# GlassyWing/yolo_deepsort

Measured on AMD Instinct MI355X. Metric: end-to-end frames/sec (detect+ReID+assoc), 608x608, higher is better.
Workload: dtype f16x3

## Files before the change

yolo_deepsort_amd/csrc/conv_bench.cpp:

```cpp
#include "conv_common.h"
#include "conv_weights.h"
#include "h16.h"

#include <algorithm>
#include <math.h>
#include <stdlib.h>
#include <string.h>

namespace yds {
namespace {

uint16_t f16_bits_saturating(float x) {
    const float xs = x * H16_A_SCALE;
    _Float16 h = (_Float16)xs;
    if (isfinite(xs) && !isfinite((float)h)) h = (_Float16)(xs > 0.f ? 65504.f : -65504.f);
    uint16_t b;
    memcpy(&b, &h, 2);
    return b;
}

struct CaseViews {
    int x_ld, x_off, y_ld, y_off, r_ld, r_off, n_split, y2_ld, y2_off;
};

struct ConvCase {
    ConvArgs a;
    ConvWeights cw;
    DevBuf<float> x, y, y2, res, raw[4];
    View y_whole, y2_whole;

    static void put(View &v, const float *host, DevBuf<float> &raw, DevBuf<float> &packed) {
        if (v.fmt == FMT_F16) {
            const size_t count = v.pixels() * v.c;
            std::vector<uint16_t> h(count);
            for (size_t i = 0; i < count; ++i) h[i] = f16_bits_saturating(host[i]);
            v.ld = fmt_slots(FMT_F16, v.c);
            packed.upload(reinterpret_cast<const float *>(h.data()), count / 2);
            YDS_HIP(hipDeviceSynchronize());
            v.p = packed.p;
            return;
        }
        raw.upload(host, v.pixels() * v.c);
        v.p = raw.p;
        if (v.fmt != FMT_H16) return;
        packed.alloc(raw.n);
        v.p = packed.p;
        launch_pack_h16(raw.p, v, nullptr);
    }
    static View slice(const View &whole, int off, int c) {
        View v = whole;
        v.p = whole.p + fmt_slots(whole.fmt, off);
        v.c = c;
        return v;
    }
    static bool h16_ok(int c, int ld, int off) { return c % 32 == 0 && ld % 32 == 0 && off % 32 == 0; }
    ConvCase(int n, int h, int w, int cin, int cout, int ksize, int stride, int act, const float *x_nhwc, const float *w_okkc, const float *bias,
             const float *res_nhwc, int res_mode, const CaseViews *vw = nullptr, float sentinel = 0.f, int fmt_x = 0, int fmt_y = 0) {
        const int pad = (ksize - 1) / 2, ho = (h + 2 * pad - ksize) / stride + 1, wo = (w + 2 * pad - ksize) / stride + 1;
        const CaseViews d = vw ? *vw : CaseViews{cin, 0, (cout + 3) / 4 * 4, 0, cout, 0, 0, 0, 0};
        const bool f16 = conv_math() == MATH_F16X3;
        const int c1 = d.n_split > 0 ? d.n_split : cout, c2 = cout - c1;
        cw.shape(cout, cin, cin, ksize, stride, pad);
        cw.upload_korder(w_okkc, bias, nullptr);
        cw.fill(a);
        a.act = act;
        View x_whole{nullptr, n, h, w, d.x_ld, d.x_ld, fmt_x == FMT_F16 ? FMT_F16 : (f16 && h16_ok(cin, d.x_ld, d.x_off)) ? FMT_H16 : FMT_F32};
        const int yfmt = fmt_y == FMT_F16 ? FMT_F16 : (f16 && h16_ok(c1, d.y_ld, d.y_off) && h16_ok(c2, d.y2_ld, d.y2_off)) ? FMT_H16 : FMT_F32;
        y_whole = View{nullptr, n, ho, wo, d.y_ld, d.y_ld, yfmt};
        if (x_nhwc) put(x_whole, x_nhwc, raw[0], x);
        else x_whole.ld = fmt_slots(x_whole.fmt, d.x_ld);
        a.x = slice(x_whole, d.x_off, cin);
        if (vw) {
            const std::vector<float> fill(y_whole.pixels() * (size_t)std::max(d.y_ld, d.y2_ld), sentinel);
            put(y_whole, fill.data(), raw[2], y);
            if (c2 > 0) {
                y2_whole = View{nullptr, n, ho, wo, d.y2_ld, d.y2_ld, yfmt};
                put(y2_whole, fill.data(), raw[3], y2);
                a.y2 = slice(y2_whole, d.y2_off, c2);
                a.n_split = c1;
            }
        } else {
            y_whole.ld = fmt_slots(yfmt, d.y_ld);
            y.alloc(y_whole.pixels() * y_whole.ld);
            y_whole.p = y.p;
        }
        a.y = slice(y_whole, d.y_off, cout);
        if (res_mode) {
            View r_whole{nullptr, n, ho, wo, d.r_ld, d.r_ld, yfmt};
            put(r_whole, res_nhwc, raw[1], res);
            a.res = slice(r_whole, d.r_off, cout);
            a.res_mode = res_mode;
        }
        YDS_HIP(hipDeviceSynchronize());
    }
};

}
}

extern "C" {

int yds_conv_bench(int n, int h, int w, int cin, int cout, int ksize, int stride, int act, int with_residual, int iters, double *avg_us,
                   int *variant) {
    YDS_API_BEGIN
    using namespace yds;
    std::vector<float> hx((size_t)n * h * w * cin), hw((size_t)cout * ksize * ksize * cin), hb(cout);
    unsigned s = 12345u;
    auto rnd = [&]() { s = s * 1664525u + 1013904223u; return ((s >> 8) & 0xffff) / 32768.f - 1.f; };
    const char *dk = getenv("YDS_BENCH_DATA");
    const int data_kind = !dk ? 0 : (!strcmp(dk, "zero") ? 1 : (!strcmp(dk, "const") ? 2 : 0));
    for (auto &v : hx) v = data_kind == 1 ? 0.f : data_kind == 2 ? 0.5f : rnd();
    for (auto &v : hw) v = data_kind == 1 ? 0.f : data_kind == 2 ? 0.03125f : rnd() * 0.05f;
    for (auto &v : hb) v = rnd();
    const int pad = (ksize - 1) / 2;
    const std::vector<float> hr(with_residual ? (size_t)n * ((h + 2 * pad - ksize) / stride + 1) * ((w + 2 * pad - ksize) / stride + 1) * cout : 0, 0.f);
    ConvCase c(n, h, w, cin, cout, ksize, stride, act, hx.data(), hw.data(), hb.data(), hr.data(), with_residual ? RES_AFTER_ACT : RES_NONE);
    if (const char *t = getenv("YDS_BENCH_TERMS")) c.a.terms = atoi(t) == 1 ? 1 : 3;
    hipStream_t st;
    YDS_HIP(hipStreamCreate(&st));
    hipEvent_t e0, e1;
    YDS_HIP(hipEventCreate(&e0)); YDS_HIP(hipEventCreate(&e1));
    int tuned = conv_autotune(c.a, st, nullptr);
    for (int i = 0; i < 3; ++i) *variant = launch_conv(c.a, st, tuned);
    YDS_HIP(hipEventRecord(e0, st));
    for (int i = 0; i < iters; ++i) launch_conv(c.a, st, tuned);
    YDS_HIP(hipEventRecord(e1, st));
    YDS_HIP(hipEventSynchronize(e1));
    float ms = 0;
    YDS_HIP(hipEventElapsedTime(&ms, e0, e1));
    *avg_us = ms * 1e3 / iters;
    (void)hipEventDestroy(e0); (void)hipEventDestroy(e1); (void)hipStreamDestroy(st);
    YDS_API_END
}

int yds_conv_run(int variant, int n, int h, int w, int cin, int cout, int ksize, int stride, int act, int res_mode, const float *x_nhwc,
                 const float *w_okkc, const float *bias, const float *res_nhwc, float *y_nchw) {
    YDS_API_BEGIN
    using namespace yds;
    if (cin % 4) fail("conv_run: input channels must be a multiple of 4");
    if (res_mode && !res_nhwc) fail("conv_run: residual mode %d without a residual tensor", res_mode);
    ConvCase c(n, h, w, cin, cout, ksize, stride, act, x_nhwc, w_okkc, bias, res_nhwc, res_mode);
    launch_conv(c.a, nullptr, variant);
    nhwc_to_host(c.a.y, y_nchw, nullptr);
    YDS_API_END
}

int yds_conv_run_view(int variant, int n, int h, int w, int cin, int cout, int ksize, int stride, int act, int res_mode, const int *view,
                      const float *x_nhwc, const float *w_okkc, const float *bias, const float *res_nhwc, float sentinel, float *y_nchw,
                      float *y2_nchw) {
    YDS_API_BEGIN
    using namespace yds;
    const CaseViews v{view[0], view[1], view[2], view[3], view[4], view[5], view[6], view[7], view[8]};
    const bool merged = v.n_split > 0;
    const int c1 = merged ? v.n_split : cout;
    if (n < 1 || h < 1 || w < 1 || cin < 4 || cout < 1 || cin % 4) fail("conv_run_view: bad shape (input channels must be a multiple of 4)");
    if (res_mode && !res_nhwc) fail("conv_run_view: residual mode %d without a residual tensor", res_mode);
    if (merged && (v.n_split >= cout || res_mode || !y2_nchw)) fail("conv_run_view: a merged launch needs 0 < n_split < cout, a second output and no residual");
    auto inside = [](int off, int c, int ld) { return off >= 0 && c > 0 && off % 4 == 0 && ld % 4 == 0 && off + c <= ld; };
    if (!inside(v.x_off, cin, v.x_ld)) fail("conv_run_view: input slice [%d, %d) does not fit %d channels (multiples of 4)", v.x_off, v.x_off + cin, v.x_ld);
    if (!inside(v.y_off, c1, v.y_ld)) fail("conv_run_view: output slice [%d, %d) does not fit %d channels (multiples of 4)", v.y_off, v.y_off + c1, v.y_ld);
    if (merged && !inside(v.y2_off, cout - c1, v.y2_ld)) fail("conv_run_view: second output slice [%d, %d) does not fit %d channels (multiples of 4)", v.y2_off, v.y2_off + cout - c1, v.y2_ld);
    if (res_mode && !inside(v.r_off, cout, v.r_ld)) fail("conv_run_view: residual slice [%d, %d) does not fit %d channels (multiples of 4)", v.r_off, v.r_off + cout, v.r_ld);
    ConvCase c(n, h, w, cin, cout, ksize, stride, act, x_nhwc, w_okkc, bias, res_nhwc, res_mode, &v, sentinel);
    const int id = variant & kVariantMask;
    if (variant < 0 || id >= kConvVariants) fail("conv_run_view: no such variant %d", variant);
    const std::vector<int> cand = conv_candidates(c.a);
    bool planned = std::find(cand.begin(), cand.end(), id) != cand.end();
    if (id == VAR_SPLITK_64x128 && conv_math() == MATH_F16X3 && !merged && conv_presplit_input(c.a)) {
        const ConvKernelArgs k = make_conv_args(c.a);
        planned = conv_splitk_applicable(k, 0) && conv_splitk_preferred(k);
    }
// ... 88 lines not shown
```

yolo_deepsort_amd/csrc/conv_common.h:

```cpp
#pragma once
#include "common.h"
#include "h16.h"

#include <algorithm>
#include <stdlib.h>
#include <type_traits>

namespace yds {

typedef float f32x16 __attribute__((ext_vector_type(16)));
typedef float f32x4 __attribute__((ext_vector_type(4)));

typedef _Float16 h8 __attribute__((ext_vector_type(8)));
typedef _Float16 h4 __attribute__((ext_vector_type(4)));
constexpr float A_SCALE = 1.f / 256.f, LO_SCALE = 2048.f;
typedef __attribute__((address_space(3))) void lds_void_t;
typedef __attribute__((address_space(1))) const void glb_void_t;
template <int N> __device__ __forceinline__ void wait_vmcnt() { asm volatile("s_waitcnt vmcnt(%0)" ::"n"(N) : "memory"); }

struct ConvKernelArgs {
    const float *x, *w, *bias, *res;
    float *y;
    int H, W, Cin, ldx;
    int Ho, Wo, Cout, ldy, ldr;
    int ksize, stride, pad;
    int K, Kpad, M;
    int act, res_mode;
    int fmt_x, fmt_y, fmt_r;
    int terms;
    int ksplit = 1;
    float *y2 = nullptr;
    int ldy2 = 0, n_split = 0;
    int tiles_m, tiles_n, xm, rm, rn;
    int gn = 1;
    int gn_req = 0;
};

constexpr int KALIGN = 32;
constexpr int STAGGER = 24;

template <int ACT> __device__ __forceinline__ float apply_act(float v) {
    if (ACT == ACT_LEAKY) return v > 0.f ? v : v * 0.1f;
    if (ACT == ACT_RELU) return v > 0.f ? v : 0.f;
    if (ACT == ACT_MISH) {
        const float e = __builtin_amdgcn_exp2f(fminf(v, 20.f) * 1.44269504088896341f);
        const float n = e * (e + 2.f);
        const float m = v * (n * __builtin_amdgcn_rcpf(n + 2.f));
        return v > 20.f ? v : m;
    }
    return v;
}

__device__ __forceinline__ bool tile_of_block(const ConvKernelArgs &p, int &tm, int &tn) {
    const int b = blockIdx.x, xcd = b & 7, idx = b >> 3;
    int lm, ln;
    if (p.gn <= 1) {
        lm = idx % p.rm;
        ln = idx / p.rm;
    } else {
        const int per = p.rm * p.gn, grp = idx / per, w = idx - grp * per;
        const int g = min(p.gn, p.rn - grp * p.gn);
        lm = w / g;
        ln = grp * p.gn + (w - lm * g);
    }
    tm = (xcd % p.xm) * p.rm + lm;
    tn = (xcd / p.xm) * p.rn + ln;
    return tm < p.tiles_m && tn < p.tiles_n;
}

inline int plan_tile_map(ConvKernelArgs &k, int BM, int BN) {
    k.tiles_m = (k.M + BM - 1) / BM;
    k.tiles_n = (k.Cout + BN - 1) / BN;
    long best = -1;
    for (int xm = 1; xm <= 8; xm *= 2) {
        int xn = 8 / xm;
        int rm = (k.tiles_m + xm - 1) / xm, rn = (k.tiles_n + xn - 1) / xn;
        long waste = (long)rm * rn * 8 - (long)k.tiles_m * k.tiles_n;
        long cost = ((long)rm * BM + (long)rn * BN) * 64 + waste * (BM + BN);
        if (best < 0 || cost < best) { best = cost; k.xm = xm; k.rm = rm; k.rn = rn; }
    }
    k.gn = std::max(1, std::min(k.gn_req, k.rn));
    return 8 * k.rm * k.rn;
}

struct FlatRows {
    int m0;
    __device__ __forceinline__ int operator()(int row) const { return m0 + row; }
};
template <int BM, int BN, int WM, int WN, int ACT, int RES, int NT, class RowMap, bool ONE_PASS, class Store>
__device__ __forceinline__ void conv_epilogue_core(const ConvKernelArgs &p, Store store, float *stage, RowMap rows, int n0, int tid) {
    constexpr int ROWS = BM / WM, LD = BN + 4, C4 = BN / 4;
    constexpr int RSTEP = NT / C4;
    static_assert(NT % C4 == 0 && C4 % 2 == 0 && ROWS % RSTEP == 0, "tile width must divide the workgroup; lane pairs share a row");
    const int wave = tid >> 6, wm = wave / WN;
    const int c4 = tid % C4, rr = tid / C4;
    const int n = n0 + c4 * 4;
    const bool n_vec = n + 3 < p.Cout;
    const bool second = p.n_split > 0 && n >= p.n_split;
    float *const y_base = second ? p.y2 : p.y;
    const int y_ld = second ? p.ldy2 : p.ldy, ny = second ? n - p.n_split : n;
    float4 bias4 = make_float4(0.f, 0.f, 0.f, 0.f);
    if (n_vec) bias4 = *reinterpret_cast<const float4 *>(p.bias + n);
    else {
        if (n < p.Cout) bias4.x = p.bias[n];
        if (n + 1 < p.Cout) bias4.y = p.bias[n + 1];
        if (n + 2 < p.Cout) bias4.z = p.bias[n + 2];
    }
    constexpr int PER_PASS = ROWS / RSTEP, NRES = RES != RES_NONE ? WM * PER_PASS : 1;
    auto sweep = [&](auto yf_c, auto rf_c) {
        constexpr int YF = decltype(yf_c)::value, RF = decltype(rf_c)::value;
        constexpr bool YH = YF == FMT_H16, RH = RF == FMT_H16, YS = YF == FMT_F16, RS = RF == FMT_F16;
        float4 rraw[NRES];
        if (RES != RES_NONE) {
#pragma unroll
            for (int q = 0; q < NRES; ++q) {
                const int m = rows((q / PER_PASS) * ROWS + rr + (q % PER_PASS) * RSTEP);
                rraw[q] = make_float4(0.f, 0.f, 0.f, 0.f);
                if (m >= 0 && m < p.M && n < p.Cout) {
                    const float *rp = p.res + (size_t)m * p.ldr;
                    if (RH) {
                        const char *g = reinterpret_cast<const char *>(rp + (n & ~31)) + (n & 31) * 2;
                        const float2 hi = *reinterpret_cast<const float2 *>(g), lo = *reinterpret_cast<const float2 *>(g + 64);
                        rraw[q] = make_float4(hi.x, hi.y, lo.x, lo.y);
                    } else if (RS) {
                        const float2 h = *reinterpret_cast<const float2 *>(reinterpret_cast<const char *>(rp) + n * 2);
                        rraw[q] = make_float4(h.x, h.y, 0.f, 0.f);
                    } else if (n_vec) {
                        rraw[q] = *reinterpret_cast<const float4 *>(rp + n);
                    } else {
                        rraw[q].x = rp[n];
                        if (n + 1 < p.Cout) rraw[q].y = rp[n + 1];
                        if (n + 2 < p.Cout) rraw[q].z = rp[n + 2];
                    }
                }
            }
        }
#pragma unroll
        for (int pass = 0; pass < WM; ++pass) {
            if (ONE_PASS ? pass == 0 : wm == pass) store(stage + (ONE_PASS ? wm * ROWS * LD : 0));
            if (!ONE_PASS || pass == 0) __syncthreads();
#pragma unroll
            for (int k2 = 0; k2 < PER_PASS; ++k2) {
                const int r = rr + k2 * RSTEP;
                const int m = rows(pass * ROWS + r);
                const bool live = m >= 0 && m < p.M && n < p.Cout;
                float4 v = *reinterpret_cast<const float4 *>(stage + (ONE_PASS ? pass * ROWS * LD : 0) + r * LD + c4 * 4);
                float rs[4] = {0.f, 0.f, 0.f, 0.f};
                if (RES != RES_NONE) {
                    const float4 t = rraw[RES != RES_NONE ? pass * PER_PASS + k2 : 0];
                    if (RH) {
                        union { float2 f; h16x4 h; } uh, ul;
                        uh.f = make_float2(t.x, t.y);
                        ul.f = make_float2(t.z, t.w);
                        h16_decode4(uh.h, ul.h, rs);
                    } else if (RS) {
                        union { float2 f; h16x4 h; } uh;
                        uh.f = make_float2(t.x, t.y);
#pragma unroll
                        for (int k = 0; k < 4; ++k) rs[k] = (float)uh.h[k] * (1.f / H16_A_SCALE);
                    } else { rs[0] = t.x; rs[1] = t.y; rs[2] = t.z; rs[3] = t.w; }
                }
                float o[4] = {v.x + bias4.x, v.y + bias4.y, v.z + bias4.z, v.w + bias4.w};
#pragma unroll
                for (int k = 0; k < 4; ++k) {
                    if (RES == RES_BEFORE_ACT) o[k] += rs[k];
                    o[k] = apply_act<ACT>(o[k]);
                    if (RES == RES_AFTER_ACT) o[k] += rs[k];
                }
                float *yp = y_base + (size_t)m * y_ld;
                if (YH) {
                    h16x4 hi, lo;
                    h16_encode4(o, hi, lo);
                    const bool odd = c4 & 1;
                    union { h16x4 h; int i[2]; } send, recv;
                    send.h = odd ? hi : lo;
                    recv.i[0] = __builtin_amdgcn_update_dpp(send.i[0], send.i[0], 0xB1, 0xF, 0xF, false);
                    recv.i[1] = __builtin_amdgcn_update_dpp(send.i[1], send.i[1], 0xB1, 0xF, 0xF, false);
                    union { h16x4 h[2]; float4 f; } out;
                    out.h[0] = odd ? recv.h : hi;
                    out.h[1] = odd ? lo : recv.h;
                    const int nq = ny & ~7;
                    char *g = reinterpret_cast<char *>(yp + (nq & ~31)) + (nq & 31) * 2 + (odd ? 64 : 0);
                    if (live) *reinterpret_cast<float4 *>(g) = out.f;
                } else if (YS) {
                    union { h16x4 h; int i[2]; } mine, other;
#pragma unroll
                    for (int k = 0; k < 4; ++k) mine.h[k] = (_Float16)(o[k] * H16_A_SCALE);
                    other.i[0] = __builtin_amdgcn_update_dpp(mine.i[0], mine.i[0], 0xB1, 0xF, 0xF, false);
                    other.i[1] = __builtin_amdgcn_update_dpp(mine.i[1], mine.i[1], 0xB1, 0xF, 0xF, false);
                    union { h16x4 h[2]; float4 f; } out;
                    out.h[0] = mine.h;
                    out.h[1] = other.h;
                    if (live && !(c4 & 1)) *reinterpret_cast<float4 *>(reinterpret_cast<char *>(yp) + ny * 2) = out.f;
                } else if (live) {
                    if (n_vec) *reinterpret_cast<float4 *>(yp + ny) = make_float4(o[0], o[1], o[2], o[3]);
                    else { yp[ny] = o[0]; if (n + 1 < p.Cout) yp[ny + 1] = o[1]; if (n + 2 < p.Cout) yp[ny + 2] = o[2]; }
                }
            }
            if (!ONE_PASS && pass + 1 < WM) __syncthreads();
        }
    };
    using F32c = std::integral_constant<int, FMT_F32>;
    using H16c = std::integral_constant<int, FMT_H16>;
    using F16c = std::integral_constant<int, FMT_F16>;
    const bool yh = p.fmt_y == FMT_H16, rh = RES != RES_NONE && p.fmt_r == FMT_H16;
    if (p.fmt_y == FMT_F16) {
        sweep(F16c{}, F16c{});
    } else if (yh) {
        if (rh) sweep(H16c{}, H16c{});
        else sweep(H16c{}, F32c{});
    } else {
        if (rh) sweep(F32c{}, H16c{});
        else sweep(F32c{}, F32c{});
    }
}
constexpr size_t conv_stage_bytes(int BM, int BN) { return (size_t)BM * (BN + 4) * sizeof(float); }

template <int BM, int BN, int WM, int WN, int ACT, int RES, int TM, int TN, int NT = 256, class RowMap = FlatRows, bool ONE_PASS = false>
__device__ __forceinline__ void conv_epilogue_rows(const ConvKernelArgs &p, f32x16 (&acc)[TM][TN], float *stage, RowMap rows, int n0, int tid) {
    constexpr int LD = BN + 4;
    const int lane = tid & 63, wn = (tid >> 6) % WN;
    const int col = lane & 31, rsel = (lane >> 5) * 4;
    auto store = [&](float *st) {
#pragma unroll
        for (int i = 0; i < TM; ++i)
#pragma unroll
            for (int j = 0; j < TN; ++j)
#pragma unroll
                for (int e = 0; e < 16; ++e)
                    st[(i * 32 + rsel + (e & 3) + 8 * (e >> 2)) * LD + wn * (BN / WN) + j * 32 + col] = acc[i][j][e];
    };
    conv_epilogue_core<BM, BN, WM, WN, ACT, RES, NT, RowMap, ONE_PASS>(p, store, stage, rows, n0, tid);
}

template <int BM, int BN, int WM, int WN, int ACT, int RES, int TM, int TN, int NT = 256, class RowMap = FlatRows, bool ONE_PASS = false>
__device__ __forceinline__ void conv_epilogue16_rows(const ConvKernelArgs &p, f32x4 (&acc)[TM][TN], float *stage, RowMap rows, int n0, int tid) {
    constexpr int LD = BN + 4;
    const int lane = tid & 63, wn = (tid >> 6) % WN;
    const int col = lane & 15, rsel = (lane >> 4) * 4;
    auto store = [&](float *st) {
#pragma unroll
        for (int i = 0; i < TM; ++i)
#pragma unroll
            for (int j = 0; j < TN; ++j)
#pragma unroll
                for (int e = 0; e < 4; ++e)
                    st[(i * 16 + rsel + e) * LD + wn * (BN / WN) + j * 16 + col] = acc[i][j][e];
    };
    conv_epilogue_core<BM, BN, WM, WN, ACT, RES, NT, RowMap, ONE_PASS>(p, store, stage, rows, n0, tid);
}
template <int BM, int BN, int WM, int WN, int ACT, int RES, int TM, int TN, int NT = 256, bool ONE_PASS = false>
__device__ __forceinline__ void conv_epilogue16(const ConvKernelArgs &p, f32x4 (&acc)[TM][TN], float *stage, int m0, int n0, int tid) {
    conv_epilogue16_rows<BM, BN, WM, WN, ACT, RES, TM, TN, NT, FlatRows, ONE_PASS>(p, acc, stage, FlatRows{m0}, n0, tid);
}

template <int BM, int BN, int WM, int WN, int ACT, int RES, int TM, int TN, int NT = 256, bool ONE_PASS = false>
__device__ __forceinline__ void conv_epilogue(const ConvKernelArgs &p, f32x16 (&acc)[TM][TN], float *stage, int m0, int n0, int tid) {
    conv_epilogue_rows<BM, BN, WM, WN, ACT, RES, TM, TN, NT, FlatRows, ONE_PASS>(p, acc, stage, FlatRows{m0}, n0, tid);
}

ConvKernelArgs make_conv_args(const ConvArgs &a);
bool conv_stem2_applicable(const ConvKernelArgs &k0, const ConvKernelArgs &k1);
void launch_conv_stem2(const ConvKernelArgs &k0, const ConvKernelArgs &k1, hipStream_t s);
bool conv_block1_applicable(const ConvKernelArgs &k2, const ConvKernelArgs &k3);
void launch_conv_block1(const ConvKernelArgs &k2, const ConvKernelArgs &k3, hipStream_t s);

template <class F> void dispatch_act_res(const ConvKernelArgs &k, F f) {
    using Linear = std::integral_constant<int, ACT_LINEAR>;
    using Leaky = std::integral_constant<int, ACT_LEAKY>;
    using Mish = std::integral_constant<int, ACT_MISH>;
    using Relu = std::integral_constant<int, ACT_RELU>;
    using None = std::integral_constant<int, RES_NONE>;
    using After = std::integral_constant<int, RES_AFTER_ACT>;
    using Before = std::integral_constant<int, RES_BEFORE_ACT>;
    switch (k.act * 4 + k.res_mode) {
        case ACT_LINEAR * 4 + RES_NONE: f(Linear{}, None{}); break;
        case ACT_LEAKY * 4 + RES_NONE: f(Leaky{}, None{}); break;
        case ACT_LEAKY * 4 + RES_AFTER_ACT: f(Leaky{}, After{}); break;
        case ACT_MISH * 4 + RES_NONE: f(Mish{}, None{}); break;
        case ACT_MISH * 4 + RES_AFTER_ACT: f(Mish{}, After{}); break;
        case ACT_RELU * 4 + RES_NONE: f(Relu{}, None{}); break;
        case ACT_RELU * 4 + RES_BEFORE_ACT: f(Relu{}, Before{}); break;
        default: fail("conv: unsupported activation/residual combination (%d, %d)", k.act, k.res_mode);
    }
}

template <auto KERN, class... Args>
void launch_conv_tiles(ConvKernelArgs k, int BM, int BN, int grid_y, int threads, size_t smem, hipStream_t s, Args... args) {
    static size_t attr_set = 0;
    if (smem > attr_set) {
        YDS_HIP(hipFuncSetAttribute(reinterpret_cast<const void *>(KERN), hipFuncAttributeMaxDynamicSharedMemorySize, (int)smem));
        attr_set = smem;
    }
    dim3 grid(plan_tile_map(k, BM, BN), grid_y);
    hipLaunchKernelGGL(KERN, grid, dim3(threads), smem, s, k, args...);
    YDS_HIP(hipGetLastError());
}

bool conv_direct_applicable(const ConvKernelArgs &k);
void launch_conv_direct(const ConvKernelArgs &k, hipStream_t s);
bool conv_pool_applicable(const ConvKernelArgs &k);
void launch_conv_pool(const ConvKernelArgs &k, hipStream_t s);

void launch_conv_f16x3_staged(ConvKernelArgs k, int tile, hipStream_t s);
void launch_conv_f16x3_dma(ConvKernelArgs k, int tile, hipStream_t s);
void launch_conv_f16x3_win(ConvKernelArgs k, int tile, hipStream_t s);
void launch_conv_f16x3_splitk(ConvKernelArgs k, int tile, hipStream_t s);
bool conv_splitk_applicable(const ConvKernelArgs &k, int tile);
bool conv_splitk_preferred(const ConvKernelArgs &k);
bool conv_win2_applicable(const ConvKernelArgs &k);
void launch_conv_win2(ConvKernelArgs k, hipStream_t s);
bool conv_win_applicable(const ConvKernelArgs &k);
void launch_conv_win(ConvKernelArgs k, int shape, hipStream_t s);
void conv_win_clock(unsigned long long *cycles_ticks, bool reset);
void conv_win16_clock(unsigned long long *cycles_ticks, bool reset);
bool conv_win16_small_applicable(const ConvKernelArgs &k);
void launch_conv_win16(ConvKernelArgs k, int shape, hipStream_t s);
void conv_win2_clock(unsigned long long *cycles_ticks, bool reset);

}
```

yolo_deepsort_amd/csrc/conv_f16x3.hip:

```cpp
#include "conv_common.h"

#include <map>
#include <mutex>

#include <math.h>
#include <string.h>

namespace yds {


constexpr int ROWB = 144;
__device__ __forceinline__ void split4(const f32x4 &v, h4 &hi, h4 &lo) {
#pragma unroll
    for (int c = 0; c < 4; ++c) {
        float xs = v[c] * A_SCALE;
        _Float16 h = (_Float16)xs;
        hi[c] = h;
        lo[c] = (_Float16)((xs - (float)h) * LO_SCALE);
    }
}

template <int BM, int BN, int ACT, int RES, int AIN>
__global__ __launch_bounds__(256, 2) void conv_igemm_f16x3(ConvKernelArgs p) {
    fp16_saturate_on();
// ... 337 lines not shown
            if (NEED_ORDER) {
                if (r < HM) read_a(next, r, false);
                else if (r < HM + HN) read_b(next, r - HM, false);
                else if (r < HM + NB) read_b(next, r - HM - HN, true);
                else if (r < NA + NB) read_a(next, r - HM - NB, true);
            } else {
                const int rb = o - B_START;
                if (r < HM) read_a(next, r, false);
                else if (r < NA) read_a(next, r - HM, true);
                else if (rb >= 0 && rb < HN) read_b(next, rb, false);
                else if (rb >= HN && rb < NB) read_b(next, rb - HN, true);
            }
        };
        auto step_head = [&](int stage) {
#pragma unroll
            for (int m = 0; m < NMQ; ++m) {
                mfma(0, 0, m);
                __builtin_amdgcn_sched_barrier(0);
                pre_op(stage, m);
                __builtin_amdgcn_sched_barrier(0);
            }
#pragma unroll
            for (int m = 0; m < NMQ; ++m) {
                mfma(0, 1, m);
                __builtin_amdgcn_sched_barrier(0);
                pre_op(stage, NMQ + m);
                __builtin_amdgcn_sched_barrier(0);
            }
            asm volatile("s_waitcnt lgkmcnt(0)" ::: "memory");
        };
        auto step_tail = [&](int stage, int next, auto refill_c, auto next_c) {
            __builtin_amdgcn_s_barrier();
            __builtin_amdgcn_sched_barrier(0);
#pragma unroll
            for (int m = 0; m < NMQ; ++m) {
                mfma(1, 0, m);
                __builtin_amdgcn_sched_barrier(0);
                post_op(stage, next, m, refill_c, next_c);
                __builtin_amdgcn_sched_barrier(0);
            }
#pragma unroll
            for (int m = 0; m < NMQ; ++m) {
                mfma(1, 1, m);
                __builtin_amdgcn_sched_barrier(0);
                post_op(stage, next, NMQ + m, refill_c, next_c);
                __builtin_amdgcn_sched_barrier(0);
            }
            if (decltype(refill_c)::value) advance_tile();
        };

        if (nk >= 3 && NS >= 3) wait_vmcnt<2 * IN>(); else if (nk >= 2) wait_vmcnt<IN>(); else wait_vmcnt<0>();
        __builtin_amdgcn_s_barrier();
#pragma unroll
        for (int i = 0; i < HM; ++i) { read_a(0, i, false); read_a(0, i, true); }
#pragma unroll
        for (int j = 0; j < HN; ++j) { read_b(0, j, false); read_b(0, j, true); }
        __builtin_amdgcn_sched_barrier(0);

        int t = 0, stage = 0;
        for (; t + NS < nk; ++t) {
            const int next = stage + 1 == NS ? 0 : stage + 1;
            step_head(stage);
            wait_vmcnt<(NS - 2) * IN>();
            step_tail(stage, next, std::true_type{}, std::true_type{});
            stage = next;
        }
        for (; t + 1 < nk; ++t) {
            const int next = stage + 1 == NS ? 0 : stage + 1;
            step_head(stage);
            if (NS >= 3 && nk - 2 - t >= 1) wait_vmcnt<(NS >= 3 ? IN : 0)>(); else wait_vmcnt<0>();
            step_tail(stage, next, std::false_type{}, std::true_type{});
            stage = next;
        }
        if (t < nk) {
            step_head(stage);
            step_tail(stage, stage, std::false_type{}, std::false_type{});
        }
        __syncthreads();
#pragma unroll
        for (int i = 0; i < TM16; ++i)
#pragma unroll
            for (int j = 0; j < TN16; ++j)
#pragma unroll
                for (int e = 0; e < 4; ++e) acc1[i][j][e] = (acc1[i][j][e] + acc2[i][j][e] * (1.f / LO_SCALE)) * (1.f / A_SCALE);
        conv_epilogue16<BM, BN, WM, WN, ACT, RES, TM16, TN16, NT, true>(p, acc1, reinterpret_cast<float *>(ring), m0, n0, tid);
    } else {
        f32x16 acc1[TM][TN], acc2[TM][TN];
#pragma unroll
        for (int i = 0; i < TM; ++i)
#pragma unroll
            for (int j = 0; j < TN; ++j)
#pragma unroll
                for (int e = 0; e < 16; ++e) { acc1[i][j][e] = 0.f; acc2[i][j][e] = 0.f; }

#pragma unroll
        for (int s = 0; s < NS - 1; ++s)
            if (s < nk) {
#pragma unroll
                for (int q = 0; q < IN; ++q) piece(s, q);
                advance_tile();
            }
        if (STAGGER && ((blockIdx.x >> 8) & 1)) __builtin_amdgcn_s_sleep(STAGGER / 4);

        const int swz = (lane >> 1) & 7, kb = lane >> 5;
        const int a_frag = (wm * (BM / WM) + (lane & 31)) * ROW, b_frag = A_BYTES + (wn * (BN / WN) + (lane & 31)) * ROW;
        int pos_hi[2], pos_lo[2];
#pragma unroll
        for (int s = 0; s < 2; ++s) { pos_hi[s] = ((2 * s + kb) ^ swz) * 16; pos_lo[s] = ((4 + 2 * s + kb) ^ swz) * 16; }

        constexpr int NF = 2 * (TM + TN);
        constexpr int NM = 3 * TM * TN;
        h8 fr[2][NF];
        auto frag_read = [&](const char *st, int s, int f) {
            const int which = f / 2, lo = f & 1;
            if (TERMS == 1 && lo) return;
            const int off = which < TM ? a_frag + which * 32 * ROW : b_frag + (which - TM) * 32 * ROW;
            fr[s][f] = *reinterpret_cast<const h8 *>(st + off + (lo ? pos_lo[s] : pos_hi[s]));
        };
        auto mfma = [&](int s, int m) {
            const int ij = m / 3, term = m % 3, i = ij / TN, j = ij % TN;
            if (TERMS == 1 && term != 0) return;
            const h8 ah = fr[s][2 * i], al = fr[s][2 * i + 1], bh = fr[s][2 * (TM + j)], bl = fr[s][2 * (TM + j) + 1];
            if (TERMS == 4) {
                if (term == 0) acc1[i][j] = __builtin_amdgcn_mfma_f32_32x32x16_f16(ah, bh, acc1[i][j], 0, 0, 0);
                else if (term == 1) acc1[i][j] = __builtin_amdgcn_mfma_f32_32x32x16_f16(al, bl, acc1[i][j], 0, 0, 0);
                return;
            }
            if (term == 0) acc1[i][j] = __builtin_amdgcn_mfma_f32_32x32x16_f16(ah, bh, acc1[i][j], 0, 0, 0);
            else if (term == 1) acc2[i][j] = __builtin_amdgcn_mfma_f32_32x32x16_f16(ah, bl, acc2[i][j], 0, 0, 0);
            else acc2[i][j] = __builtin_amdgcn_mfma_f32_32x32x16_f16(al, bh, acc2[i][j], 0, 0, 0);
        };
        constexpr int P0 = IN < NM - 4 ? IN : NM - 4;
        constexpr int F0 = NM - P0 < NF ? NM - P0 : NF;
        static_assert(IN - P0 + NF - F0 <= NM, "not enough MFMA slots for the interleaved memory instructions");
        auto frag_order = [&](int k) {
            if (k < 2) return k;
            if (k < 4) return 2 * TM + (k - 2);
            const int r = k - 4, nb = 2 * (TN - 1);
            return r < nb ? 2 * TM + 2 + r : 2 + (r - nb);
        };
        auto step = [&](int t, auto refill_c) {
            constexpr bool REFILL = decltype(refill_c)::value;
            const char *st = ring + (t % NS) * STAGE;
            const int fill_stage = (t + NS - 1) % NS;
#pragma unroll
            for (int f = 0; f < NF; ++f) frag_read(st, 0, f);
            __builtin_amdgcn_sched_barrier(0);
#pragma unroll
            for (int m = 0; m < NM; ++m) {
                mfma(0, m);
                __builtin_amdgcn_sched_barrier(0);
                if (m < P0) { if (REFILL) piece(fill_stage, m); }
                else if (m - P0 < F0) frag_read(st, 1, frag_order(m - P0));
                __builtin_amdgcn_sched_barrier(0);
            }
#pragma unroll
            for (int m = 0; m < NM; ++m) {
                mfma(1, m);
                __builtin_amdgcn_sched_barrier(0);
                if (m < NF - F0) frag_read(st, 1, frag_order(F0 + m));
                else if (REFILL && P0 + (m - (NF - F0)) < IN) piece(fill_stage, P0 + (m - (NF - F0)));
                __builtin_amdgcn_sched_barrier(0);
            }
            if (REFILL) advance_tile();
        };
        int t = 0;
        for (; t + NS - 1 < nk; ++t) {
            wait_vmcnt<(NS - 2) * IN>();
// ... 185 lines not shown
```

yolo_deepsort_amd/csrc/conv_win16.hip:

```cpp
#include "conv_win_common.h"

namespace yds {
namespace {

template <int BM, int BN, int WM, int WN, int ACT, int RES>
__global__ __launch_bounds__(WM * WN * 64, WM * WN == 8 ? 1 : 2) void conv3x3_f16x3_win16(ConvKernelArgs p, int wrows, int nbuf) {
    fp16_saturate_on();
    constexpr int NW = WM * WN, NT = NW * 64;
    static_assert(NW == 8 || NW == 4, "eight waves (one workgroup per CU) or four (two)");
    constexpr int RW = BM / WM, CW = BN / WN;
    constexpr int TM = RW / 16, TN = CW / 16;
    constexpr int HM = TM / 2, HN = TN / 2;
    static_assert(TM % 2 == 0 && TN % 2 == 0, "the wave tile splits into quadrants");
    constexpr int B_STAGE = BN * ROW;
    constexpr int B_INST = BN / (8 * NW);
    extern __shared__ __attribute__((aligned(16))) char smem[];
    const int WB = wrows * ROW;
    char *bring = smem + nbuf * WB;
    const int zoff = nbuf * WB + NSB * B_STAGE;

    const int tid = threadIdx.x;
    const int lane = tid & 63, wave = __builtin_amdgcn_readfirstlane(tid >> 6);
    const int wm = wave / WN, wn = wave % WN;
    int m0, n0;
// ... 72 lines not shown
    auto tap_addr = [&](int g, int tap) {
        const int shift = (tap / 3) * W + (tap % 3);
        const int wbase = (g & 1) * WB;
        int rj = r0 + shift;
        asm volatile("" : "+v"(rj));
#pragma unroll
        for (int i = 0; i < TM; ++i) {
            const bool ok = (okbits[i / 3] >> (9 * (i % 3) + tap)) & 1u;
            const int j = rj + i * 16;
            a_hi[i] = ok ? wbase + j * ROW + ((kq ^ ((j >> 1) & 7)) << 4) : zoff + (kq << 4);
        }
    };
    auto step = [&](auto tap_c, int g, auto last_c) {
        constexpr int TAP = decltype(tap_c)::value;
        constexpr bool LAST = decltype(last_c)::value;
        constexpr bool REFILL = !(LAST && TAP + 2 > 8);
        constexpr bool NEXT = !(LAST && TAP == 8);
        constexpr int TAP1 = (TAP + 1) % 9, TAP2 = (TAP + 2) % 9;
        const int g1 = TAP + 1 >= 9 ? g + 1 : g, g2 = TAP + 2 >= 9 ? g + 1 : g;
        const char *bst = bring + (TAP % NSB) * B_STAGE, *bst1 = bring + ((TAP + 1) % NSB) * B_STAGE;
        auto dma = [&](int o) {
            if (o == 0) { if (!LAST && TAP < APW) a_piece(g + 1, TAP); }
            else if (o - 1 < B_INST) { if (REFILL) b_piece(g2, TAP2, (TAP + 2) % NSB, o - 1); }
        };
        constexpr int NA = 2 * HM, NB = 2 * HN;
#pragma unroll
        for (int m = 0; m < NMQ; ++m) {
            mfma(0, 0, m);
            __builtin_amdgcn_sched_barrier(0);
            if (m < NB) frag_read(bst, 1, NA + m);
            __builtin_amdgcn_sched_barrier(0);
        }
#pragma unroll
        for (int m = 0; m < NMQ; ++m) {
            mfma(0, 1, m);
            __builtin_amdgcn_sched_barrier(0);
            if (m < NA) frag_read(bst, 1, m);
            __builtin_amdgcn_sched_barrier(0);
        }
        wait_vmcnt<0>();
        __builtin_amdgcn_s_barrier();
        if (NEXT) tap_addr(g1, TAP1);
        __builtin_amdgcn_sched_barrier(0);
#pragma unroll
        for (int m = 0; m < NMQ; ++m) {
            mfma(1, 0, m);
            __builtin_amdgcn_sched_barrier(0);
            if (m <= B_INST) dma(m);
            else if (NEXT && m - 1 - B_INST < NA) frag_read(bst1, 0, m - 1 - B_INST);
            __builtin_amdgcn_sched_barrier(0);
        }
        static_assert(1 + B_INST + NA <= NMQ, "Q10 holds the DMA pieces and the A fragments");
#pragma unroll
        for (int m = 0; m < NMQ; ++m) {
            mfma(1, 1, m);
            __builtin_amdgcn_sched_barrier(0);
            if (NEXT && m < NB) frag_read(bst1, 0, NA + m);
            __builtin_amdgcn_sched_barrier(0);
        }
    };
    auto group = [&](int g, auto last_c) { for_each_tap(step, g, last_c); };

    for (int k = 0; k < (npieces + NW - 1) / NW; ++k) a_piece(0, k);
#pragma unroll
    for (int b = 0; b < B_INST; ++b) b_piece(0, 0, 0, b);
#pragma unroll
    for (int b = 0; b < B_INST; ++b) b_piece(0, 1, 1, b);
    wait_vmcnt<B_INST>();
    __syncthreads();
    tap_addr(0, 0);
#pragma unroll
    for (int f = 0; f < NRH; ++f) frag_read(bring, 0, f);
    __builtin_amdgcn_sched_barrier(0);

    for (int g = 0; g + 1 < G; ++g) group(g, std::false_type{});
    group(G - 1, std::true_type{});

    __syncthreads();
#pragma unroll
    for (int i = 0; i < TM; ++i)
#pragma unroll
        for (int j = 0; j < TN; ++j)
#pragma unroll
            for (int e = 0; e < 4; ++e) acc1[i][j][e] = (acc1[i][j][e] + acc2[i][j][e] * (1.f / LO_SCALE)) * (1.f / A_SCALE);
    conv_epilogue16<BM, BN, WM, WN, ACT, RES, TM, TN, NT, true>(p, acc1, reinterpret_cast<float *>(smem), m0, n0, tid);
    clk.end();
}

template <int BM, int BN, int WM, int WN, int ACT, int RES> void launch_inst_win16(ConvKernelArgs k, hipStream_t s) {
    const int nbuf = win_buffers(k.Cin, 32);
    const WinPlan plan = win_plan(WIN128, BM, BN, WM * WN, k.W, nbuf);
    launch_conv_tiles<conv3x3_f16x3_win16<BM, BN, WM, WN, ACT, RES>>(k, BM, BN, 1, WM * WN * 64, plan.launch_bytes, s, plan.wrows, nbuf);
}

constexpr int SMALL_BM = 128, SMALL_BN = 64, SMALL_NW = 4;

}

void conv_win16_clock(unsigned long long *cycles_ticks, bool reset) { clock_probe_read(cycles_ticks, reset); }

bool conv_win16_small_applicable(const ConvKernelArgs &k) {
    if (!conv_win_applicable(k) || k.Cout > SMALL_BN) return false;
    const WinPlan plan = win_plan(WIN128, SMALL_BM, SMALL_BN, SMALL_NW, k.W, win_buffers(k.Cin, 32));
    return plan.prefetch_fits && plan.launch_bytes <= 80 * 1024;
}

void launch_conv_win16(ConvKernelArgs k, int shape, hipStream_t s) {
    if (shape != 0 && shape != 1 && !conv_win16_small_applicable(k)) fail("conv: the 128x64 window-resident tile needs a 3x3 stride-1 layer with a pre-split input, at most 64 filters and W <= 43");
    dispatch_act_res(k, [&](auto A, auto R) {
        if (shape == 0) launch_inst_win16<256, 128, 4, 2, A, R>(k, s);
        else if (shape == 1) launch_inst_win16<256, 64, 8, 1, A, R>(k, s);
        else launch_inst_win16<SMALL_BM, SMALL_BN, SMALL_NW, 1, A, R>(k, s);
    });
}

}
```

yolo_deepsort_amd/csrc/h16.h:

```cpp
#pragma once
#include <hip/hip_runtime.h>

namespace yds {

enum TensorFmt { FMT_F32 = 0, FMT_H16 = 1, FMT_F16 = 2 };
__host__ __device__ inline int fmt_slots(int fmt, int c) { return fmt == FMT_F16 ? c / 2 : c; }

constexpr float H16_A_SCALE = 1.f / 256.f, H16_LO_SCALE = 2048.f;

typedef _Float16 h16x4 __attribute__((ext_vector_type(4)));

__device__ __forceinline__ void fp16_saturate_on() { asm volatile("s_setreg_imm32_b32 hwreg(HW_REG_MODE, 23, 1), 1"); }

__device__ __forceinline__ void h16_encode4(const float v[4], h16x4 &hi, h16x4 &lo) {
#pragma unroll
    for (int c = 0; c < 4; ++c) {
        float xs = v[c] * H16_A_SCALE;
        _Float16 h = (_Float16)xs;
        hi[c] = h;
        lo[c] = (_Float16)((xs - (float)h) * H16_LO_SCALE);
    }
}

__device__ __forceinline__ void h16_encode4_scaled(const float xs[4], h16x4 &hi, h16x4 &lo) {
#pragma unroll
    for (int c = 0; c < 4; ++c) {
        _Float16 h = (_Float16)xs[c];
        hi[c] = h;
        lo[c] = (_Float16)((xs[c] - (float)h) * H16_LO_SCALE);
    }
}

__device__ __forceinline__ void h16_decode4(const h16x4 &hi, const h16x4 &lo, float v[4]) {
#pragma unroll
    for (int c = 0; c < 4; ++c) v[c] = ((float)hi[c] + (float)lo[c] * (1.f / H16_LO_SCALE)) * (1.f / H16_A_SCALE);
}

__device__ __forceinline__ void h16_load4(const float *pixel, int c, float v[4]) {
    const char *g = reinterpret_cast<const char *>(pixel + (c & ~31)) + (c & 31) * 2;
    h16x4 hi = *reinterpret_cast<const h16x4 *>(g), lo = *reinterpret_cast<const h16x4 *>(g + 64);
    h16_decode4(hi, lo, v);
}
__device__ __forceinline__ void h16_store4(float *pixel, int c, const float v[4]) {
    char *g = reinterpret_cast<char *>(pixel + (c & ~31)) + (c & 31) * 2;
    h16x4 hi, lo;
    h16_encode4(v, hi, lo);
    *reinterpret_cast<h16x4 *>(g) = hi;
    *reinterpret_cast<h16x4 *>(g + 64) = lo;
}

__device__ __forceinline__ void f16_load4(const float *pixel, int c, float v[4]) {
    const h16x4 h = *reinterpret_cast<const h16x4 *>(reinterpret_cast<const char *>(pixel) + c * 2);
#pragma unroll
    for (int k = 0; k < 4; ++k) v[k] = (float)h[k] * (1.f / H16_A_SCALE);
}
__device__ __forceinline__ void f16_store4(float *pixel, int c, const float v[4]) {
    h16x4 h;
#pragma unroll
    for (int k = 0; k < 4; ++k) h[k] = (_Float16)(v[k] * H16_A_SCALE);
    *reinterpret_cast<h16x4 *>(reinterpret_cast<char *>(pixel) + c * 2) = h;
}

__device__ __forceinline__ void load4(const float *pixel, int c, int fmt, float v[4]) {
    if (fmt == FMT_H16) h16_load4(pixel, c, v);
    else if (fmt == FMT_F16) f16_load4(pixel, c, v);
    else {
        float4 t = *reinterpret_cast<const float4 *>(pixel + c);
        v[0] = t.x; v[1] = t.y; v[2] = t.z; v[3] = t.w;
    }
}
__device__ __forceinline__ void store4(float *pixel, int c, int fmt, const float v[4]) {
    if (fmt == FMT_H16) h16_store4(pixel, c, v);
    else if (fmt == FMT_F16) f16_store4(pixel, c, v);
    else *reinterpret_cast<float4 *>(pixel + c) = make_float4(v[0], v[1], v[2], v[3]);
}

}
```

Before: 1688.

## Add fast full-tile conv epilogue working in scaled domain with wider stores

Adds a specialised epilogue path for full interior tiles that skips per-element bounds checks, processes 8 channels per thread for h16 outputs with full 16-byte stores, and precomputes residual addresses. It also keeps values in the A_SCALE domain through bias, residual and leaky activation, which removes the multiply-by-scale and divide-by-scale pairs around the h16 encode and decode. The bench also picks an h16 residual format when it is valid. This adds template variants and code size, and the scaled leaky path uses a max-based form.

```diff
diff --git a/yolo_deepsort_amd/csrc/conv_bench.cpp b/yolo_deepsort_amd/csrc/conv_bench.cpp
--- a/yolo_deepsort_amd/csrc/conv_bench.cpp
+++ b/yolo_deepsort_amd/csrc/conv_bench.cpp
@@ -86,7 +86,8 @@
         }
         a.y = slice(y_whole, d.y_off, cout);
         if (res_mode) {
-            View r_whole{nullptr, n, ho, wo, d.r_ld, d.r_ld, yfmt};
+            const int rfmt = yfmt == FMT_F16 ? FMT_F16 : (f16 && h16_ok(cout, d.r_ld, d.r_off)) ? FMT_H16 : FMT_F32;
+            View r_whole{nullptr, n, ho, wo, d.r_ld, d.r_ld, rfmt};
             put(r_whole, res_nhwc, raw[1], res);
             a.res = slice(r_whole, d.r_off, cout);
             a.res_mode = res_mode;
diff --git a/yolo_deepsort_amd/csrc/conv_common.h b/yolo_deepsort_amd/csrc/conv_common.h
--- a/yolo_deepsort_amd/csrc/conv_common.h
+++ b/yolo_deepsort_amd/csrc/conv_common.h
@@ -87,9 +87,125 @@
     int m0;
     __device__ __forceinline__ int operator()(int row) const { return m0 + row; }
 };
-template <int BM, int BN, int WM, int WN, int ACT, int RES, int NT, class RowMap, bool ONE_PASS, class Store>
+constexpr bool conv_epilogue_scaled(bool fast, int act) { return fast && act != ACT_MISH; }
+template <int ACT, bool SC> __device__ __forceinline__ float conv_epilogue_act(float o) {
+    if (SC && ACT == ACT_LEAKY) return fmaxf(o, o * 0.1f);
+    return apply_act<ACT>(o);
+}
+
+template <int BM, int BN, int WM, int WN, int ACT, int RES, int NT, bool SC, class Store>
+__device__ __forceinline__ void conv_epilogue_full(const ConvKernelArgs &p, Store store, float *stage, int m0, int n0, int tid) {
+    constexpr int ROWS = BM / WM, LD = BN + 4;
+    const int wm = (tid >> 6) / WN;
+    const bool second = p.n_split > 0 && n0 >= p.n_split;
+    const int y_ld = second ? p.ldy2 : p.ldy, ny0 = second ? n0 - p.n_split : n0;
+    char *const y_tile = reinterpret_cast<char *>((second ? p.y2 : p.y) + (size_t)m0 * y_ld);
+    const char *const r_tile = RES != RES_NONE ? reinterpret_cast<const char *>(p.res + (size_t)m0 * p.ldr) : nullptr;
+    auto sweep = [&](auto yh_c, auto rh_c) {
+        constexpr bool YH = decltype(yh_c)::value, RH = decltype(rh_c)::value;
+        constexpr int CH = YH ? 8 : 4, Q = CH / 4;
+        constexpr int CT = BN / CH, RSTEP = NT / CT, NIT = BM / RSTEP;
+        static_assert(NT % CT == 0 && BM % RSTEP == 0, "tile width must divide the workgroup");
+        const int c = tid % CT, rr = tid / CT;
+        const int n = n0 + c * CH, ny = ny0 + c * CH;
+        auto chan_off = [](bool h16, int ch) { return h16 ? (unsigned)(ch & ~31) * 4u + (unsigned)(ch & 31) * 2u : (unsigned)ch * 4u; };
+        const unsigned y_off = (unsigned)(rr * y_ld) * 4u + chan_off(YH, ny), y_step = (unsigned)(RSTEP * y_ld) * 4u;
+        float bias[CH];
+#pragma unroll
+        for (int q = 0; q < Q; ++q) {
+            const float4 b = *reinterpret_cast<const float4 *>(p.bias + n + q * 4);
+            bias[q * 4] = b.x; bias[q * 4 + 1] = b.y; bias[q * 4 + 2] = b.z; bias[q * 4 + 3] = b.w;
+        }
+        if (SC) {
+#pragma unroll
+            for (int k = 0; k < CH; ++k) bias[k] *= A_SCALE;
+        }
+        union ResRow { float4 f[Q]; float2 d[2 * Q]; _Float16 h[2 * CH]; float v[CH]; };
+        ResRow rraw[RES != RES_NONE ? NIT : 1];
+        if (RES != RES_NONE) {
+            const unsigned r_off = (unsigned)(rr * p.ldr) * 4u + chan_off(RH, n), r_step = (unsigned)(RSTEP * p.ldr) * 4u;
+#pragma unroll
+            for (int it = 0; it < NIT; ++it) {
+                const char *g = r_tile + (r_off + (unsigned)it * r_step);
+                if (RH && CH == 8) {
+                    rraw[it].f[0] = *reinterpret_cast<const float4 *>(g);
+                    rraw[it].f[Q - 1] = *reinterpret_cast<const float4 *>(g + 64);
+                } else if (RH) {
+                    rraw[it].d[0] = *reinterpret_cast<const float2 *>(g);
+                    rraw[it].d[1] = *reinterpret_cast<const float2 *>(g + 64);
+                } else {
+#pragma unroll
+                    for (int q = 0; q < Q; ++q) rraw[it].f[q] = *reinterpret_cast<const float4 *>(g + q * 16);
+                }
+            }
+        }
+        store(stage + wm * ROWS * LD);
+        __syncthreads();
+        const float *st = stage + rr * LD + c * CH;
+#pragma unroll
+        for (int it = 0; it < NIT; ++it) {
+            float o[CH];
+#pragma unroll
+            for (int q = 0; q < Q; ++q) {
+                const float4 v = *reinterpret_cast<const float4 *>(st + it * RSTEP * LD + q * 4);
+                o[q * 4] = v.x + bias[q * 4]; o[q * 4 + 1] = v.y + bias[q * 4 + 1]; o[q * 4 + 2] = v.z + bias[q * 4 + 2]; o[q * 4 + 3] = v.w + bias[q * 4 + 3];
+            }
+#pragma unroll
+            for (int k = 0; k < CH; ++k) {
+                float rs = 0.f;
+                if (RES != RES_NONE) {
+                    const ResRow &t = rraw[RES != RES_NONE ? it : 0];
+                    if (RH) {
+                        rs = (float)t.h[k] + (float)t.h[CH + k] * (1.f / H16_LO_SCALE);
+                        if (!SC) rs *= 1.f / H16_A_SCALE;
+                    } else rs = SC ? t.v[k] * A_SCALE : t.v[k];
+                }
+                if (RES == RES_BEFORE_ACT) o[k] += rs;
+                o[k] = conv_epilogue_act<ACT, SC>(o[k]);
+                if (RES == RES_AFTER_ACT) o[k] += rs;
+            }
+            char *g = y_tile + (y_off + (unsigned)it * y_step);
+            if (YH) {
+                union { h16x4 h[2]; float4 f; } hi, lo;
+#pragma unroll
+                for (int q = 0; q < 2; ++q) {
+                    if (SC) h16_encode4_scaled(o + q * 4, hi.h[q], lo.h[q]);
+                    else h16_encode4(o + q * 4, hi.h[q], lo.h[q]);
+                }
+                *reinterpret_cast<float4 *>(g) = hi.f;
+                *reinterpret_cast<float4 *>(g + 64) = lo.f;
+            } else {
+                if (SC) {
+#pragma unroll
+                    for (int k = 0; k < 4; ++k) o[k] *= 1.f / A_SCALE;
+                }
+                *reinterpret_cast<float4 *>(g) = make_float4(o[0], o[1], o[2], o[3]);
+            }
+        }
+    };
+    const bool yh = p.fmt_y == FMT_H16, rh = RES != RES_NONE && p.fmt_r == FMT_H16;
+    if (yh) {
+        if (rh) sweep(std::true_type{}, std::true_type{});
+        else sweep(std::true_type{}, std::false_type{});
+    } else {
+        if (rh) sweep(std::false_type{}, std::true_type{});
+        else sweep(std::false_type{}, std::false_type{});
+    }
+}
+
+template <int BM, int BN, int WM, int WN, int ACT, int RES, int NT, class RowMap, bool ONE_PASS, bool FAST, class Store>
 __device__ __forceinline__ void conv_epilogue_core(const ConvKernelArgs &p, Store store, float *stage, RowMap rows, int n0, int tid) {
     constexpr int ROWS = BM / WM, LD = BN + 4, C4 = BN / 4;
+    constexpr bool SC = conv_epilogue_scaled(FAST, ACT);
+    if constexpr (FAST) {
+        static_assert(ONE_PASS && std::is_same<RowMap, FlatRows>::value, "the full-tile sweep reads a whole staged tile of consecutive pixels");
+        const int m0 = rows(0);
+        const bool split_inside = p.n_split > n0 && p.n_split < n0 + BN;
+        if (m0 + BM <= p.M && n0 + BN <= p.Cout && !split_inside && p.fmt_y != FMT_F16) {
+            conv_epilogue_full<BM, BN, WM, WN, ACT, RES, NT, SC>(p, store, stage, m0, n0, tid);
+            return;
+        }
+    }
     constexpr int RSTEP = NT / C4;
     static_assert(NT % C4 == 0 && C4 % 2 == 0 && ROWS % RSTEP == 0, "tile width must divide the workgroup; lane pairs share a row");
     const int wave = tid >> 6, wm = wave / WN;
@@ -106,6 +222,7 @@
         if (n + 1 < p.Cout) bias4.y = p.bias[n + 1];
         if (n + 2 < p.Cout) bias4.z = p.bias[n + 2];
     }
+    if (SC) { bias4.x *= A_SCALE; bias4.y *= A_SCALE; bias4.z *= A_SCALE; bias4.w *= A_SCALE; }
     constexpr int PER_PASS = ROWS / RSTEP, NRES = RES != RES_NONE ? WM * PER_PASS : 1;
     auto sweep = [&](auto yf_c, auto rf_c) {
         constexpr int YF = decltype(yf_c)::value, RF = decltype(rf_c)::value;
@@ -152,25 +269,30 @@
                         union { float2 f; h16x4 h; } uh, ul;
                         uh.f = make_float2(t.x, t.y);
                         ul.f = make_float2(t.z, t.w);
-                        h16_decode4(uh.h, ul.h, rs);
+                        if (SC) h16_decode4_scaled(uh.h, ul.h, rs);
+                        else h16_decode4(uh.h, ul.h, rs);
                     } else if (RS) {
                         union { float2 f; h16x4 h; } uh;
                         uh.f = make_float2(t.x, t.y);
 #pragma unroll
-                        for (int k = 0; k < 4; ++k) rs[k] = (float)uh.h[k] * (1.f / H16_A_SCALE);
-                    } else { rs[0] = t.x; rs[1] = t.y; rs[2] = t.z; rs[3] = t.w; }
+                        for (int k = 0; k < 4; ++k) rs[k] = SC ? (float)uh.h[k] : (float)uh.h[k] * (1.f / H16_A_SCALE);
+                    } else {
+                        rs[0] = t.x; rs[1] = t.y; rs[2] = t.z; rs[3] = t.w;
+                        if (SC) { rs[0] *= A_SCALE; rs[1] *= A_SCALE; rs[2] *= A_SCALE; rs[3] *= A_SCALE; }
+                    }
                 }
                 float o[4] = {v.x + bias4.x, v.y + bias4.y, v.z + bias4.z, v.w + bias4.w};
 #pragma unroll
                 for (int k = 0; k < 4; ++k) {
                     if (RES == RES_BEFORE_ACT) o[k] += rs[k];
-                    o[k] = apply_act<ACT>(o[k]);
+                    o[k] = conv_epilogue_act<ACT, SC>(o[k]);
                     if (RES == RES_AFTER_ACT) o[k] += rs[k];
                 }
                 float *yp = y_base + (size_t)m * y_ld;
                 if (YH) {
                     h16x4 hi, lo;
-                    h16_encode4(o, hi, lo);
+                    if (SC) h16_encode4_scaled(o, hi, lo);
+                    else h16_encode4(o, hi, lo);
                     const bool odd = c4 & 1;
                     union { h16x4 h; int i[2]; } send, recv;
                     send.h = odd ? hi : lo;
@@ -185,7 +307,7 @@
                 } else if (YS) {
                     union { h16x4 h; int i[2]; } mine, other;
 #pragma unroll
-                    for (int k = 0; k < 4; ++k) mine.h[k] = (_Float16)(o[k] * H16_A_SCALE);
+                    for (int k = 0; k < 4; ++k) mine.h[k] = SC ? (_Float16)o[k] : (_Float16)(o[k] * H16_A_SCALE);
                     other.i[0] = __builtin_amdgcn_update_dpp(mine.i[0], mine.i[0], 0xB1, 0xF, 0xF, false);
                     other.i[1] = __builtin_amdgcn_update_dpp(mine.i[1], mine.i[1], 0xB1, 0xF, 0xF, false);
                     union { h16x4 h[2]; float4 f; } out;
@@ -193,6 +315,10 @@
                     out.h[1] = other.h;
                     if (live && !(c4 & 1)) *reinterpret_cast<float4 *>(reinterpret_cast<char *>(yp) + ny * 2) = out.f;
                 } else if (live) {
+                    if (SC) {
+#pragma unroll
+                        for (int k = 0; k < 4; ++k) o[k] *= 1.f / A_SCALE;
+                    }
                     if (n_vec) *reinterpret_cast<float4 *>(yp + ny) = make_float4(o[0], o[1], o[2], o[3]);
                     else { yp[ny] = o[0]; if (n + 1 < p.Cout) yp[ny + 1] = o[1]; if (n + 2 < p.Cout) yp[ny + 2] = o[2]; }
                 }
@@ -230,10 +356,10 @@
                 for (int e = 0; e < 16; ++e)
                     st[(i * 32 + rsel + (e & 3) + 8 * (e >> 2)) * LD + wn * (BN / WN) + j * 32 + col] = acc[i][j][e];
     };
-    conv_epilogue_core<BM, BN, WM, WN, ACT, RES, NT, RowMap, ONE_PASS>(p, store, stage, rows, n0, tid);
-}
-
-template <int BM, int BN, int WM, int WN, int ACT, int RES, int TM, int TN, int NT = 256, class RowMap = FlatRows, bool ONE_PASS = false>
+    conv_epilogue_core<BM, BN, WM, WN, ACT, RES, NT, RowMap, ONE_PASS, false>(p, store, stage, rows, n0, tid);
+}
+
+template <int BM, int BN, int WM, int WN, int ACT, int RES, int TM, int TN, int NT = 256, class RowMap = FlatRows, bool ONE_PASS = false, bool FAST = false>
 __device__ __forceinline__ void conv_epilogue16_rows(const ConvKernelArgs &p, f32x4 (&acc)[TM][TN], float *stage, RowMap rows, int n0, int tid) {
     constexpr int LD = BN + 4;
     const int lane = tid & 63, wn = (tid >> 6) % WN;
@@ -247,11 +373,11 @@
                 for (int e = 0; e < 4; ++e)
                     st[(i * 16 + rsel + e) * LD + wn * (BN / WN) + j * 16 + col] = acc[i][j][e];
     };
-    conv_epilogue_core<BM, BN, WM, WN, ACT, RES, NT, RowMap, ONE_PASS>(p, store, stage, rows, n0, tid);
-}
-template <int BM, int BN, int WM, int WN, int ACT, int RES, int TM, int TN, int NT = 256, bool ONE_PASS = false>
+    conv_epilogue_core<BM, BN, WM, WN, ACT, RES, NT, RowMap, ONE_PASS, FAST>(p, store, stage, rows, n0, tid);
+}
+template <int BM, int BN, int WM, int WN, int ACT, int RES, int TM, int TN, int NT = 256, bool ONE_PASS = false, bool FAST = false>
 __device__ __forceinline__ void conv_epilogue16(const ConvKernelArgs &p, f32x4 (&acc)[TM][TN], float *stage, int m0, int n0, int tid) {
-    conv_epilogue16_rows<BM, BN, WM, WN, ACT, RES, TM, TN, NT, FlatRows, ONE_PASS>(p, acc, stage, FlatRows{m0}, n0, tid);
+    conv_epilogue16_rows<BM, BN, WM, WN, ACT, RES, TM, TN, NT, FlatRows, ONE_PASS, FAST>(p, acc, stage, FlatRows{m0}, n0, tid);
 }
 
 template <int BM, int BN, int WM, int WN, int ACT, int RES, int TM, int TN, int NT = 256, bool ONE_PASS = false>
diff --git a/yolo_deepsort_amd/csrc/conv_f16x3.hip b/yolo_deepsort_amd/csrc/conv_f16x3.hip
--- a/yolo_deepsort_amd/csrc/conv_f16x3.hip
+++ b/yolo_deepsort_amd/csrc/conv_f16x3.hip
@@ -443,8 +443,11 @@
 #pragma unroll
             for (int j = 0; j < TN16; ++j)
 #pragma unroll
-                for (int e = 0; e < 4; ++e) acc1[i][j][e] = (acc1[i][j][e] + acc2[i][j][e] * (1.f / LO_SCALE)) * (1.f / A_SCALE);
-        conv_epilogue16<BM, BN, WM, WN, ACT, RES, TM16, TN16, NT, true>(p, acc1, reinterpret_cast<float *>(ring), m0, n0, tid);
+                for (int e = 0; e < 4; ++e) {
+                    const float os = acc1[i][j][e] + acc2[i][j][e] * (1.f / LO_SCALE);
+                    acc1[i][j][e] = conv_epilogue_scaled(true, ACT) ? os : os * (1.f / A_SCALE);
+                }
+        conv_epilogue16<BM, BN, WM, WN, ACT, RES, TM16, TN16, NT, true, true>(p, acc1, reinterpret_cast<float *>(ring), m0, n0, tid);
     } else {
         f32x16 acc1[TM][TN], acc2[TM][TN];
 #pragma unroll
diff --git a/yolo_deepsort_amd/csrc/conv_win16.hip b/yolo_deepsort_amd/csrc/conv_win16.hip
--- a/yolo_deepsort_amd/csrc/conv_win16.hip
+++ b/yolo_deepsort_amd/csrc/conv_win16.hip
@@ -178,8 +178,11 @@
 #pragma unroll
         for (int j = 0; j < TN; ++j)
 #pragma unroll
-            for (int e = 0; e < 4; ++e) acc1[i][j][e] = (acc1[i][j][e] + acc2[i][j][e] * (1.f / LO_SCALE)) * (1.f / A_SCALE);
-    conv_epilogue16<BM, BN, WM, WN, ACT, RES, TM, TN, NT, true>(p, acc1, reinterpret_cast<float *>(smem), m0, n0, tid);
+            for (int e = 0; e < 4; ++e) {
+                const float os = acc1[i][j][e] + acc2[i][j][e] * (1.f / LO_SCALE);
+                acc1[i][j][e] = conv_epilogue_scaled(true, ACT) ? os : os * (1.f / A_SCALE);
+            }
+    conv_epilogue16<BM, BN, WM, WN, ACT, RES, TM, TN, NT, true, true>(p, acc1, reinterpret_cast<float *>(smem), m0, n0, tid);
     clk.end();
 }
 
diff --git a/yolo_deepsort_amd/csrc/h16.h b/yolo_deepsort_amd/csrc/h16.h
--- a/yolo_deepsort_amd/csrc/h16.h
+++ b/yolo_deepsort_amd/csrc/h16.h
@@ -34,6 +34,11 @@
 __device__ __forceinline__ void h16_decode4(const h16x4 &hi, const h16x4 &lo, float v[4]) {
 #pragma unroll
     for (int c = 0; c < 4; ++c) v[c] = ((float)hi[c] + (float)lo[c] * (1.f / H16_LO_SCALE)) * (1.f / H16_A_SCALE);
+}
+
+__device__ __forceinline__ void h16_decode4_scaled(const h16x4 &hi, const h16x4 &lo, float xs[4]) {
+#pragma unroll
+    for (int c = 0; c < 4; ++c) xs[c] = (float)hi[c] + (float)lo[c] * (1.f / H16_LO_SCALE);
 }
 
 __device__ __forceinline__ void h16_load4(const float *pixel, int c, float v[4]) {
```

New measurement: 1736 (median of 6 runs). 1.03x the previous value.
